# humanlongevity/tredparse

Measured on AMD Instinct MI355X. Metric: sample x TRED genotypes/sec at 30x 150bp, higher is better.
Workload: dtype int32 (SW) + f64 (likelihood)

## Files before the change

tredparse_amd/csrc/capi.hip:

```cpp
#include <algorithm>
#include <cstdarg>
#include <cstdio>
#include <cmath>
#include <cstdlib>
#include <cstring>
#include <ctime>
#include <string>
#include <vector>

#include <unistd.h>

#include "tredgpu_internal.h"
#include "inflater_internal.h"

using namespace tredgpu;

namespace {

struct Buf {
    void* p = nullptr;
    size_t cap = 0;
};

std::string g_create_error;

}

struct tredgpu_ctx {
    int device = 0;
    hipStream_t stream = nullptr;
    std::string err;
    std::vector<LadderDesc> h_ladders;
    Buf d_ladders, d_seq;
    int max_ladder_units = 0;
    Buf d_model;
    bool have_model = false;
    Buf ws_quads, ws_counter, ws_drop, ws_grid, ws_stats, ws_perm, ws_class, ws_gdesc, ws_gtile, ws_gctr, ws_ucnt, ws_bins, ws_kde, ws_best, ws_cnt;
    int* h_pin = nullptr;
    hipEvent_t sync_ev = nullptr;
    size_t grid_pool_bytes = GRID_POOL_BYTES;
    std::vector<Buf> st;
    struct PinBlock { uint8_t* p; size_t cap, used; };
    std::vector<PinBlock> pin;
    struct PinOut { void* host; const void* pinned; size_t bytes; };
    std::vector<PinOut> pin_out;
    struct Timer {
        std::vector<std::pair<hipEvent_t, hipEvent_t>> pool;
        size_t used = 0;
        int64_t launches = 0;
        double total_ms = 0;
    } timers[7];
};

namespace {

int fail(tredgpu_ctx* c, int code, const char* fmt, ...) {
    char buf[512];
    va_list ap;
    va_start(ap, fmt);
    vsnprintf(buf, sizeof buf, fmt, ap);
    va_end(ap);
    if (c) c->err = buf; else g_create_error = buf;
    return code;
}

int hip_rc(tredgpu_ctx* c, hipError_t e, const char* what) {
    return e == hipSuccess ? 0 : fail(c, -10, "%s: %s", what, hipGetErrorString(e));
}

#define HIPRC(c, expr) hip_rc((c), (expr), #expr)
#define HIPCHK(c, expr)                          \
    do {                                         \
        if (int rc_ = HIPRC(c, expr)) return rc_; \
    } while (0)

void timer_flush(tredgpu_ctx::Timer& t) {
    for (size_t i = 0; i < t.used; ++i) {
        float ms = 0;
        if (hipEventElapsedTime(&ms, t.pool[i].first, t.pool[i].second) == hipSuccess) {
            t.total_ms += ms;
            t.launches += 1;
        }
    }
    t.used = 0;
}

struct ScopedTimer {
    tredgpu_ctx* c;
    tredgpu_ctx::Timer& t;
    hipEvent_t stop = nullptr;
    ScopedTimer(tredgpu_ctx* c_, int which) : c(c_), t(c_->timers[which]) {
        if (t.used >= 256) {
            (void)hipStreamSynchronize(c->stream);
            timer_flush(t);
        }
        if (t.used == t.pool.size()) {
// ... 283 lines not shown
    if (!c || !out) return -2;
    HIPCHK(c, hipSetDevice(c->device));
    for (int i = 0; i < 8; ++i) out[i] = 0;
    if (c->ws_stats.p) {
        std::vector<uint64_t> slots((size_t)SW_STAT_SLOTS * 8);
        HIPCHK(c, hipMemcpyAsync(slots.data(), c->ws_stats.p, slots.size() * sizeof(uint64_t), hipMemcpyDeviceToHost, c->stream));
        HIPCHK(c, stream_sync(c));
        for (int k = 0; k < SW_STAT_SLOTS; ++k)
            for (int i = 0; i < 8; ++i) out[i] += slots[(size_t)k * 8 + i];
    }
    HIPCHK(c, stream_sync(c));
    return 0;
}

int tredgpu_get_timing(tredgpu_ctx* c, int which, int64_t* launches, double* total_ms) {
    if (!c) return -2;
    if (which < 0 || which > 6) return fail(c, -2, "which must be one of TREDGPU_KERNEL_*");
    HIPCHK(c, hipSetDevice(c->device));
    HIPCHK(c, stream_sync(c));
    timer_flush(c->timers[which]);
    if (launches) *launches = c->timers[which].launches;
    if (total_ms) *total_ms = c->timers[which].total_ms;
    return 0;
}

int tredgpu_set_ladders(tredgpu_ctx* c, int32_t n, const char* const* prefix, const char* const* repeat,
                        const char* const* suffix, const int32_t* max_units) {
    if (!c) return -2;
    if (n < 0 || (n > 0 && (!prefix || !repeat || !suffix || !max_units))) return fail(c, -2, "bad ladder arguments");
    HIPCHK(c, hipSetDevice(c->device));
    std::vector<uint32_t> seq;
    auto append = [&seq](const std::vector<int8_t>& v) {
        const int off = (int)seq.size();
        seq.resize(seq.size() + (v.size() + 7) / 8 + 1, 0x44444444u);
        for (size_t i = 0; i < v.size(); ++i) {
            uint32_t& w = seq[off + i / 8];
            w = (w & ~(0xFu << ((i % 8) * 4))) | ((uint32_t)v[i] << ((i % 8) * 4));
        }
        return off;
    };
    std::vector<LadderDesc> lad((size_t)n);
    int max_u = 0;
    for (int i = 0; i < n; ++i) {
        std::vector<int8_t> P, Rp, S;
        encode(prefix[i], P);
        encode(repeat[i], Rp);
        encode(suffix[i], S);
        const int mu = max_units[i];
        LadderDesc& d = lad[i];
        memset(&d, 0, sizeof d);
        if (mu < 0) return fail(c, -2, "ladder %d: negative max_units", i);
        if (mu == 0) {
            if (P.empty() || P.size() > TREDGPU_MAX_TEMPLATE_LEN)
                return fail(c, -2, "ladder %d: reference length %zu not in [1,%d]", i, P.size(), TREDGPU_MAX_TEMPLATE_LEN);
            d.alen[0] = (int)P.size();
            d.trunk_off[0] = append(P);
            d.branch_off[0] = append(std::vector<int8_t>());
            d.period = 1;
            d.max_units = 0;
            d.n_strands = 1;
            continue;
        }
        if (Rp.empty()) return fail(c, -2, "ladder %d: empty repeat", i);
        const size_t T = P.size() + S.size() + Rp.size() * (size_t)mu;
        if (T > TREDGPU_MAX_TEMPLATE_LEN)
            return fail(c, -2, "ladder %d: longest template %zu exceeds %d", i, T, TREDGPU_MAX_TEMPLATE_LEN);
        const std::vector<int8_t> Pr = revcomp(P), Rr = revcomp(Rp), Sr = revcomp(S);
        const std::vector<int8_t>* A[2] = {&P, &Sr};
        const std::vector<int8_t>* Rep[2] = {&Rp, &Rr};
        const std::vector<int8_t>* B[2] = {&S, &Pr};
        for (int s = 0; s < 2; ++s) {
            d.alen[s] = (int)A[s]->size();
            d.blen[s] = (int)B[s]->size();
            std::vector<int8_t> trunk(*A[s]);
            for (int k = 0; k < mu; ++k) trunk.insert(trunk.end(), Rep[s]->begin(), Rep[s]->end());
            d.trunk_off[s] = append(trunk);
            d.branch_off[s] = append(*B[s]);
        }
        d.period = (int)Rp.size();
        d.max_units = mu;
        d.n_strands = 2;
        d.kmer_ok = 1;
        for (int s = 0; s < 2; ++s) {
            std::vector<uint32_t> bits(128, 0u);
            for (int u = 1; u <= mu; ++u) {
                std::vector<int8_t> t(*A[s]);
                for (int k = 0; k < u; ++k) t.insert(t.end(), Rep[s]->begin(), Rep[s]->end());
                t.insert(t.end(), B[s]->begin(), B[s]->end());
                for (size_t i = 0; i + 6 <= t.size(); ++i) {
                    uint32_t code = 0;
                    int wild[6], nw = 0;
                    for (int k = 0; k < 6; ++k) {
                        if (t[i + k] > 3) wild[nw++] = k;
                        else code |= (uint32_t)(t[i + k] & 3) << (2 * k);
                    }
                    for (uint32_t f = 0; f < (1u << (2 * nw)); ++f) {
                        uint32_t cf = code;
                        for (int j = 0; j < nw; ++j) cf |= ((f >> (2 * j)) & 3u) << (2 * wild[j]);
                        bits[cf >> 5] |= 1u << (cf & 31);
                    }
                }
            }
            d.kmer_off[s] = (int)seq.size();
            seq.insert(seq.end(), bits.begin(), bits.end());
        }
        max_u = std::max(max_u, mu);
    }
    seq.resize(seq.size() + 4, 0x44444444u);
    int rc;
    if ((rc = ensure(c, c->d_ladders, lad.size() * sizeof(LadderDesc)))) return rc;
    if ((rc = ensure(c, c->d_seq, seq.size() * sizeof(uint32_t)))) return rc;
    HIPCHK(c, stream_sync(c));
    if (n) HIPCHK(c, hipMemcpy(c->d_ladders.p, lad.data(), lad.size() * sizeof(LadderDesc), hipMemcpyHostToDevice));
    HIPCHK(c, hipMemcpy(c->d_seq.p, seq.data(), seq.size() * sizeof(uint32_t), hipMemcpyHostToDevice));
    c->h_ladders.swap(lad);
    c->max_ladder_units = max_u;
    return 0;
}

int tredgpu_set_model(tredgpu_ctx* c, const double* step_pdf, const double* stutter_w, double gc, double score) {
    if (!c) return -2;
    if (!step_pdf || !stutter_w) return fail(c, -2, "model arrays are NULL");
    HIPCHK(c, hipSetDevice(c->device));
    std::vector<ModelConst> mbuf(1);
    ModelConst& m = mbuf[0];
    memcpy(m.step, step_pdf, sizeof m.step);
    memcpy(m.w, stutter_w, sizeof m.w);
    m.gc = gc;
    m.score = score;
    m.small = std::exp(-10.0);
    m.really_small = std::exp(-100.0);
    m.logsmall = std::log(m.small);
    for (int n = 0; n < GRID_LFACT; ++n) m.lfact[n] = std::lgamma((double)n + 1);
    int rc;
    if ((rc = ensure(c, c->d_model, sizeof m))) return rc;
    HIPCHK(c, stream_sync(c));
    HIPCHK(c, hipMemcpy(c->d_model.p, &m, sizeof m, hipMemcpyHostToDevice));
    c->have_model = true;
    return 0;
}

int64_t tredgpu_pack_reads(const char* seqs, const int64_t* seq_off, int64_t n_reads, uint32_t* packed_out,
                           int64_t* word_off_out, int32_t* len_out) {
    if (n_reads < 0 || (n_reads > 0 && (!seqs || !seq_off))) return -2;
    int64_t w = 0;
    for (int64_t r = 0; r < n_reads; ++r) {
        const int64_t L = seq_off[r + 1] - seq_off[r];
        if (L < 0 || L > 0x7fffffff) return -2;
        const int64_t nb = (L + 15) >> 4, nm = (L + 31) >> 5;
        if (word_off_out) word_off_out[r] = w;
        if (len_out) len_out[r] = (int32_t)L;
        if (packed_out) {
            uint32_t* rec = packed_out + w;
            for (int64_t k = 0; k < nb + nm; ++k) rec[k] = 0;
            const char* s = seqs + seq_off[r];
            for (int64_t i = 0; i < L; ++i) {
                const int code = base_code(s[i]);
                if (code == 4) rec[nb + (i >> 5)] |= 1u << (i & 31);
                else rec[i >> 4] |= (uint32_t)code << ((i & 15) * 2);
            }
        }
        w += nb + nm;
    }
    if (word_off_out) word_off_out[n_reads] = w;
    return w;
}


static int run_sw_device(tredgpu_ctx* c, const uint32_t* packed, const int64_t* read_off, const int32_t* read_len,
                         int64_t n_reads, const int32_t* unit_read_off, const int32_t* unit_ladder,
                         int32_t n_units, const tredgpu_sw_params* p, int max_len, uint8_t* out_tag,
                         int16_t* out_h, int16_t* out_score, int16_t* out_dump, int32_t dump_templates) {
    if (n_reads == 0 || n_units == 0) return 0;
    const int n_ladders = (int)c->h_ladders.size();
    const int64_t max_quads = sw_max_quads(n_reads, n_ladders);
    int rc;
    if ((rc = ensure(c, c->ws_quads, (size_t)max_quads * sizeof(Quad)))) return rc;
    if ((rc = ensure(c, c->ws_counter, 64))) return rc;
    SwArgs a;
    a.packed = packed;
    a.read_off = read_off;
    a.read_len = read_len;
    a.unit_read_off = unit_read_off;
    a.unit_ladder = unit_ladder;
    a.ladders = (const LadderDesc*)c->d_ladders.p;
    a.seqw = (const uint32_t*)c->d_seq.p;
    a.quads = (const Quad*)c->ws_quads.p;
    a.n_quads = (const int32_t*)c->ws_counter.p;
    a.out_tag = out_tag;
    a.out_h = out_h;
    a.out_score = out_score;
    a.out_dump = out_dump;
    a.dump_templates = dump_templates;
    a.n_units = n_units;
    a.n_ladders = n_ladders;
    a.max_rows = 16 * rows_for(max_len);
    a.p = *p;
    a.stats = nullptr;
    if ((rc = ensure(c, c->ws_perm, (size_t)n_reads * sizeof(int32_t)))) return rc;
    if ((rc = ensure(c, c->ws_class, (size_t)n_reads))) return rc;
    a.perm = (const int32_t*)c->ws_perm.p;
    if ((rc = ensure(c, c->ws_ucnt, sw_unit_cnt_bytes(n_units)))) return rc;
    if ((rc = ensure(c, c->ws_bins, sw_bin_bytes(n_ladders)))) return rc;
    if ((rc = ensure(c, c->ws_best, (size_t)n_reads * sizeof(int32_t)))) return rc;
    if ((rc = ensure(c, c->ws_cnt, (size_t)n_reads * sizeof(int32_t)))) return rc;
    a.best = (int32_t*)c->ws_best.p;
    if (c->ws_stats.p == nullptr) {
        if ((rc = ensure(c, c->ws_stats, SW_STAT_SLOTS * 8 * sizeof(unsigned long long)))) return rc;
        HIPCHK(c, hipMemsetAsync(c->ws_stats.p, 0, SW_STAT_SLOTS * 8 * sizeof(unsigned long long), c->stream));
    }
    a.stats = (unsigned long long*)c->ws_stats.p;
    const int rows = rows_for(max_len);
    auto build_quads = [&](int pass) {
        return launch_build_quads(a, pass, rows, (uint8_t*)c->ws_class.p, (int32_t*)c->ws_cnt.p, (int32_t*)c->ws_perm.p,
                                  (Quad*)c->ws_quads.p, (int32_t*)c->ws_counter.p, (int32_t*)c->ws_ucnt.p,
                                  (int32_t*)c->ws_bins.p, n_ladders, max_quads, c->stream);
    };
    HIPCHK(c, build_quads(0));
    {
        ScopedTimer tm(c, TREDGPU_KERNEL_SW);
        bool generic = false;
        bool two_strands = false;
        for (const LadderDesc& d : c->h_ladders) {
            for (int s2 = 0; s2 < d.n_strands; ++s2) generic = generic || (d.max_units > 0 && d.blen[s2] * p->match >= 30);
            two_strands = two_strands || d.n_strands >= 2;
        }
        HIPCHK(c, launch_sw_ladder(a, rows, generic, max_quads, c->stream));
        if (out_dump == nullptr && two_strands) {
            HIPCHK(c, build_quads(1));
            HIPCHK(c, launch_sw_ladder(a, rows, generic, max_quads, c->stream));
        }
    }
    return 0;
}

int tredgpu_sw_classify(tredgpu_ctx* c, int mem, const uint32_t* packed, const int64_t* read_off,
                        const int32_t* read_len, int64_t n_reads, const int32_t* unit_read_off,
                        const int32_t* unit_ladder, int32_t n_units, const tredgpu_sw_params* params,
                        uint8_t* out_tag, int16_t* out_h, int16_t* out_score, int16_t* out_dump,
                        int32_t dump_templates) {
    if (!c) return -2;
    int rc;
    if ((rc = check_sw_params(c, params))) return rc;
    if (n_reads < 0 || n_units < 0) return fail(c, -2, "negative sizes");
    if (n_reads > 0 && (!packed || !read_off || !read_len || !unit_read_off || !unit_ladder || !out_tag || !out_h || !out_score))
        return fail(c, -2, "NULL array argument");
    if (c->h_ladders.empty()) return fail(c, -4, "no ladders registered (tredgpu_set_ladders)");
    if (out_dump && dump_templates <= 0) return fail(c, -2, "dump_templates must be > 0 with out_dump");
    HIPCHK(c, hipSetDevice(c->device));
    int max_len = params->max_read_len;
    if (mem == TREDGPU_MEM_DEVICE) {
        if (max_len <= 0) max_len = TREDGPU_ASSUMED_READ_LEN;
        if (out_dump) HIPCHK(c, hipMemsetAsync(out_dump, 0xFF, (size_t)n_reads * dump_templates * 6 * sizeof(int16_t), c->stream));
        return run_sw_device(c, packed, read_off, read_len, n_reads, unit_read_off, unit_ladder, n_units, params,
                             max_len, out_tag, out_h, out_score, out_dump, dump_templates);
    }
    if (mem != TREDGPU_MEM_HOST) return fail(c, -2, "mem must be TREDGPU_MEM_HOST or TREDGPU_MEM_DEVICE");
    if (n_reads == 0) return 0;
    if (unit_read_off[0] != 0 || unit_read_off[n_units] != n_reads) return fail(c, -2, "unit_read_off must span [0,n_reads]");
    for (int g = 0; g < n_units; ++g) {
        if (unit_read_off[g + 1] < unit_read_off[g]) return fail(c, -2, "unit_read_off not monotone at %d", g);
        if (unit_ladder[g] < 0 || unit_ladder[g] >= (int)c->h_ladders.size()) return fail(c, -2, "unit %d: ladder %d not registered", g, unit_ladder[g]);
    }
    if ((rc = host_max_len(c, params, read_len, n_reads, &max_len))) return rc;
    const uint32_t* d_packed; const int64_t* d_off; const int32_t* d_len; const int32_t* d_uoff; const int32_t* d_ulad;
    uint8_t* d_tag; int16_t* d_h; int16_t* d_score; int16_t* d_dump = nullptr;
    const size_t n = (size_t)n_reads, g = (size_t)n_units, dump_n = out_dump ? n * dump_templates * 6 : 0;
    const std::vector<Staged> list = {
        arr_in(d_packed, packed, (size_t)read_off[n_reads]), arr_in(d_off, read_off, n + 1), arr_in(d_len, read_len, n),
        arr_in(d_uoff, unit_read_off, g + 1), arr_in(d_ulad, unit_ladder, g),
        arr_out(d_tag, out_tag, n), arr_out(d_h, out_h, n), arr_out(d_score, out_score, n),
        out_dump ? arr_out(d_dump, out_dump, dump_n) : absent,
    };
    rc = stage(c, list);
    if (!rc && out_dump) rc = HIPRC(c, hipMemsetAsync(d_dump, 0xFF, dump_n * sizeof(int16_t), c->stream));
    if (!rc) rc = run_sw_device(c, d_packed, d_off, d_len, n_reads, d_uoff, d_ulad, n_units, params, max_len, d_tag, d_h,
                                d_score, d_dump, dump_templates);
    return finish(c, list, rc);
}

int tredgpu_tally(tredgpu_ctx* c, int mem, const uint8_t* tag, const int16_t* h, int64_t n_reads,
                  const int32_t* unit_read_off, int32_t n_units, const int32_t* read_pair_id, int32_t hist_stride,
                  int32_t* full_cnt, int32_t* pref_cnt, int32_t* rept_cnt) {
    if (!c) return -2;
    if (n_reads < 0 || n_units < 0 || hist_stride <= 0) return fail(c, -2, "bad sizes");
    if (n_units > 0 && (!unit_read_off || !full_cnt || !pref_cnt || !rept_cnt)) return fail(c, -2, "NULL array argument");
    if (n_reads > 0 && (!tag || !h)) return fail(c, -2, "NULL array argument");
    HIPCHK(c, hipSetDevice(c->device));
    int rc;
// ... 402 lines not shown
```

tredparse_amd/csrc/sw_ladder.hip:

```cpp
#include "tredgpu_internal.h"

namespace tredgpu {
namespace {

constexpr int KSH = 18;
constexpr int KONE = 1 << KSH;
constexpr int PAYMASK = KONE - 1;
constexpr int NEG = -(1 << 30);
constexpr int PADNEG = -64 * KONE;

template <int CTRL>
__device__ __forceinline__ int dpp_row_shr(int old, int x) {
    return __builtin_amdgcn_update_dpp(old, x, CTRL, 0xF, 0xF, false);
}

__device__ __forceinline__ int add3_vsv(int v0, int s1, int v2) {
    int d;
    asm("v_add3_u32 %0, %1, %2, %3" : "=v"(d) : "v"(v0), "s"(s1), "v"(v2));
    return d;
}
__device__ __forceinline__ int add_sv(int s0, int v1) {
    int d;
    asm("v_add_u32 %0, %1, %2" : "=v"(d) : "s"(s0), "v"(v1));
    return d;
}
__device__ __forceinline__ int max3(int a, int b, int c) { return max(max(a, b), c); }

__device__ __forceinline__ int row_scan_max(int x) {
    x = max(x, dpp_row_shr<0x111>(x, x));
    x = max(x, dpp_row_shr<0x112>(x, x));
    x = max(x, dpp_row_shr<0x114>(x, x));
    x = max(x, dpp_row_shr<0x118>(x, x));
    return x;
}

template <int CTRL>
__device__ __forceinline__ void pair_step(int& k, int& s) {
    const int tk = dpp_row_shr<CTRL>(k, k);
    const int ts = dpp_row_shr<CTRL>(s, s);
    const bool c = tk > k;
    k = c ? tk : k;
    s = c ? ts : s;
}

template <int R>
struct Rows {
    int S[4][R];
    int rowc0;
};

struct Track {
    int bestkey;
    int beststart;
    int ceil;
};

__device__ __forceinline__ int row_excl_scan_max(int x) {
    constexpr int IMIN = -2147483647 - 1;
    x = max(x, dpp_row_shr<0x111>(IMIN, x));
    x = max(x, dpp_row_shr<0x112>(IMIN, x));
    x = max(x, dpp_row_shr<0x114>(IMIN, x));
    x = max(x, dpp_row_shr<0x118>(IMIN, x));
    return dpp_row_shr<0x111>(NEG, x);
}

__device__ __forceinline__ int row_max_all(int x) {
    constexpr int IMIN = -2147483647 - 1;
    x = max(x, __builtin_amdgcn_update_dpp(IMIN, x, 0x121, 0xF, 0xF, false));
    x = max(x, __builtin_amdgcn_update_dpp(IMIN, x, 0x122, 0xF, 0xF, false));
    x = max(x, __builtin_amdgcn_update_dpp(IMIN, x, 0x124, 0xF, 0xF, false));
    x = max(x, __builtin_amdgcn_update_dpp(IMIN, x, 0x128, 0xF, 0xF, false));
    return x;
}

__device__ __forceinline__ int row_scan_max_fused(int x) {
    constexpr int IMIN = -2147483647 - 1;
    x = max(x, dpp_row_shr<0x111>(IMIN, x));
    x = max(x, dpp_row_shr<0x112>(IMIN, x));
    x = max(x, dpp_row_shr<0x114>(IMIN, x));
    x = max(x, dpp_row_shr<0x118>(IMIN, x));
    return x;
}

__device__ __forceinline__ int row_excl_scan_max_e10(int x, int* E, const int* q, int before) {
    int fin;
    asm("v_max_i32 %2, %2, %12\n\t"
        "v_max_i32 %3, %3, %13\n\t"
        "v_max_i32_dpp %0, %0, %0 row_shr:1 row_mask:0xf bank_mask:0xf\n\t"
        "v_max_i32 %4, %4, %14\n\t"
        "v_max_i32 %5, %5, %15\n\t"
        "v_max_i32_dpp %0, %0, %0 row_shr:2 row_mask:0xf bank_mask:0xf\n\t"
        "v_max_i32 %6, %6, %16\n\t"
// ... 244 lines not shown

__device__ __forceinline__ int lane_now() {
    int l;
    asm volatile("v_mbcnt_lo_u32_b32 %0, -1, 0\n\tv_mbcnt_hi_u32_b32 %0, -1, %0" : "=v"(l));
    return l;
}

#ifndef SW_WAVES_R4
#define SW_WAVES_R4 6
#endif
#ifndef SW_WAVES_R7
#define SW_WAVES_R7 6
#endif
#ifndef SW_WAVES_R10
#define SW_WAVES_R10 4
#endif
#ifndef SW_WAVES_R16
#define SW_WAVES_R16 3
#endif
#ifndef SW_WAVES_R20
#define SW_WAVES_R20 2
#endif
#ifndef SW_WAVES_R32
#define SW_WAVES_R32 1
#endif
template <int R, int W, bool GENERIC>
__global__ __launch_bounds__(64, W) void sw_cont_kernel(SwArgs a) {
    constexpr int PS = 64;
    __shared__ __attribute__((aligned(8))) int wbuf[(3 * R + 2) * PS + 2 * PS];
    const int lane = threadIdx.x;
    const int64_t q = (int64_t)blockIdx.x;
    const int nq = *a.n_quads;
    if (q >= nq) return;
    const int q_ladder = __builtin_amdgcn_readfirstlane(a.quads[q].ladder);
    const int q_first = __builtin_amdgcn_readfirstlane(a.quads[q].first);
    const int q_strands = __builtin_amdgcn_readfirstlane(a.quads[q].strands);
    const int q_count = __builtin_amdgcn_readfirstlane(a.quads[q].count);
    const LadderDesc* ld = a.ladders + q_ladder;
    const int period = __builtin_amdgcn_readfirstlane(ld->period);
    const int max_units = __builtin_amdgcn_readfirstlane(ld->max_units);
    const int n_strands = __builtin_amdgcn_readfirstlane(ld->n_strands);

    const int job = lane >> 4, jl = lane & 15;
    const bool valid = job < q_count;
    int L, row0;
    bool too_long;
    int best;
    {
        const int64_t rd = valid ? (int64_t)a.perm[q_first + job] : 0;
        L = valid ? a.read_len[rd] : 0;
        best = valid ? a.best[rd] : -1;
        too_long = L > 16 * R;
        if (too_long) L = 0;
        row0 = jl * R;
    }
    auto read_base = [&]() -> int64_t {
        const int jb = lane_now() >> 4;
        return jb < q_count ? a.read_off[a.perm[q_first + jb]] : 0;
    };
    const int mK = a.p.match * KONE;
    const int xK = -a.p.mismatch * KONE;
    const int geK = a.p.gap_extend * KONE;
    const int c0 = (a.p.gap_open - a.p.gap_extend) * KONE;
    const int flank = a.p.flank;
    const bool full_dump = GENERIC && a.out_dump != nullptr;
    int* const wb = wbuf + lane;
    int* const rowbuf = wb + (2 * R + 2) * PS;

    const int mu_rept = a.p.clip ? (L + period - 1) / period : max_units;

    uint32_t cnt_cols = 0, cnt_ends = 0;

    const int kmer_thr = min(a.p.mismatch, a.p.gap_open) >= 5 * a.p.match ? (30 + a.p.match - 1) / a.p.match - 5 : 0;
    const int floor_key = (full_dump ? 0 : 29) << KSH | PAYMASK;

    for (int s = 0; s < n_strands; ++s) {
        if (!((q_strands >> s) & 1)) continue;
        const int trunk_w = __builtin_amdgcn_readfirstlane(ld->trunk_off[s]);
        const int alen = __builtin_amdgcn_readfirstlane(ld->alen[s]);
        const int blen = __builtin_amdgcn_readfirstlane(ld->blen[s]);
        const int ncols = alen + period * max_units;
        int kcap = 1 << 20;
        if constexpr (R >= 5 && 2 * R + 10 <= 32) if (!full_dump && kmer_thr > 0 && __builtin_amdgcn_readfirstlane(ld->kmer_ok) != 0) {
            const uint32_t* bm = a.seqw + __builtin_amdgcn_readfirstlane(ld->kmer_off[s]);
            uint32_t pk_s, nk_s;
            {
                int L_s = L, row0_s = row0;
                asm volatile("" : "+v"(L_s), "+v"(row0_s));
                uint64_t code2;
                uint32_t nmask;
                load_rows<R>(a, read_base(), L_s, row0_s, code2, nmask);
                const int n_real = min(max(L_s - row0_s, 0), R);
                pk_s = (uint32_t)code2 & ((1u << (2 * R)) - 1u);
                nk_s = (nmask | ~((1u << n_real) - 1u)) & ((1u << R) - 1u);
            }
            const uint32_t pk_n = (uint32_t)__builtin_amdgcn_update_dpp(0, (int)pk_s, 0x101, 0xF, 0xF, false);
            const uint32_t nk_n = (uint32_t)__builtin_amdgcn_update_dpp(0x3FF, (int)nk_s, 0x101, 0xF, 0xF, false);
            const uint32_t comb = pk_s | ((pk_n & 0x3FFu) << (2 * R));
            const uint32_t ncomb = nk_s | ((nk_n & 0x1Fu) << R);
            int cnt = 0;
#pragma unroll
            for (int r = 0; r < R; ++r) {
                const uint32_t win = (comb >> (2 * r)) & 0xFFFu;
                const bool has_n = ((ncomb >> r) & 0x3Fu) != 0;
                const bool in_read = row0 + r + 5 < L;
                const uint32_t word = bm[win >> 5];
                cnt += in_read && (has_n || ((word >> (win & 31)) & 1u));
            }
            cnt += dpp_row_shr<0x111>(0, cnt);
            cnt += dpp_row_shr<0x112>(0, cnt);
            cnt += dpp_row_shr<0x114>(0, cnt);
            cnt += dpp_row_shr<0x118>(0, cnt);
            kcap = (cnt + 5) * a.p.match;
            if (__builtin_amdgcn_ballot_w64(valid && jl == 15 && cnt >= kmer_thr) == 0) continue;
        }
        const int cap = min(kcap, L * a.p.match);
        auto still_open = [&](int un) {
            const int min_score = max(min(L, alen + period * un + blen) >> 1, 30);
            return max(min_score, (best >> 12) + 1) <= cap;
        };
        if (!full_dump && __builtin_amdgcn_ballot_w64(valid && jl == 15 && still_open(max_units > 0 ? 1 : 0)) == 0) continue;

        Rows<R> J;
        int H[R], E[R];
        const bool has_suffix = max_units > 0 && blen > 0;
        if (has_suffix) {
            build_profile<R>(J, a, read_base(), L, row0, true, mK, xK, geK);
            const int branch_w = __builtin_amdgcn_readfirstlane(ld->branch_off[s]);
            const int ln = lane_now();
            const int bw = ln < ((blen + 7) >> 3) ? (int)a.seqw[branch_w + ln] : 0;
            int D[R];
#pragma unroll
            for (int r = 0; r < R; ++r) { H[r] = NEG; E[r] = NEG; }
            for (int y = 0; y + 1 < blen; ++y) {
                const int s_fresh = (y << 9) + y * geK - 2 * geK;
                switch (letter_from(bw, blen - 1 - y)) {
                    case 0: sweep_column_free<R, 0>(J, H, E, s_fresh, geK, c0); break;
                    case 1: sweep_column_free<R, 1>(J, H, E, s_fresh, geK, c0); break;
                    case 2: sweep_column_free<R, 2>(J, H, E, s_fresh, geK, c0); break;
                    case 3: sweep_column_free<R, 3>(J, H, E, s_fresh, geK, c0); break;
                    default: sweep_column_free<R, 4>(J, H, E, s_fresh, geK, c0); break;
                }
            }
            {
                const int y = blen - 1;
                const int s_fresh = (y << 9) + y * geK - 2 * geK;
                switch (letter_from(bw, 0)) {
                    case 0: match_column<R, 0>(J, H, D, s_fresh, geK); break;
                    case 1: match_column<R, 1>(J, H, D, s_fresh, geK); break;
                    case 2: match_column<R, 2>(J, H, D, s_fresh, geK); break;
                    case 3: match_column<R, 3>(J, H, D, s_fresh, geK); break;
                    default: match_column<R, 4>(J, H, D, s_fresh, geK); break;
                }
            }
            mirror_up<R>(D, 0, wb, PS);
            mirror_up<R>(E, c0, wb + R * PS, PS);
#pragma unroll
            for (int r = 0; r < R; ++r) wb[r * PS] = max(wb[r * PS], wb[(R + r) * PS] - c0);
            cnt_cols += (uint32_t)blen << 16;
        }
        build_profile<R>(J, a, read_base(), L, row0, false, mK, xK, geK);
        const int row0g = row0 * geK;
        Track T;
        const bool with_sfx = GENERIC && has_suffix && (full_dump || blen * a.p.match >= 30);
        if (with_sfx) {
            const int branch_w = __builtin_amdgcn_readfirstlane(ld->branch_off[s]);
            const int ln = lane_now();
            const int bw = ln < ((blen + 7) >> 3) ? (int)a.seqw[branch_w + ln] : 0;
            column_start<R>(J, H, E, geK);
            T.bestkey = floor_key; T.beststart = 0; T.ceil = floor_key;
            for (int j = 0; j < blen; ++j) sweep_letter<R>(letter_from(bw, j), J, H, E, T, j, row0, geK, c0, row0g, rowbuf);
            resolve_best<R>(T, row0, row0g, geK, rowbuf);
            int sk = T.bestkey, ss = T.beststart;
            pair_step<0x111>(sk, ss);
            pair_step<0x112>(sk, ss);
            pair_step<0x114>(sk, ss);
            pair_step<0x118>(sk, ss);
            wb[(2 * R) * PS] = sk;
            wb[(2 * R + 1) * PS] = ss;
        }
        const int ln_t = lane_now();
        const int tw = ln_t < ((ncols + 7) >> 3) ? (int)a.seqw[trunk_w + ln_t] : 0;
        column_start<R>(J, H, E, geK);
        T.bestkey = floor_key; T.beststart = 0; T.ceil = floor_key;
        int next_end = max_units > 0 ? alen + period - 1 : alen - 1;
        int u = max_units > 0 ? 1 : 0;
        auto template_end = [&](int col) -> bool {
            const bool comb = blen > 0;
            const int Tlen = alen + period * u + blen;
            next_end += period;
            int bk, bs;
            if (comb) {
                long long* const slot = reinterpret_cast<long long*>(wbuf + (3 * R + 2) * PS) + lane_now();
#pragma unroll
                for (int r0 = 0; r0 < R; r0 += END_CHUNK<R>) {
                    int wh[END_CHUNK<R>], we[END_CHUNK<R>];
// ... 76 lines not shown
                const int k = max_units > 0 ? 2 * (u - 1) + s : 0;
                if (k < a.dump_templates) {
                    int16_t* d = a.out_dump + ((int64_t)a.perm[q_first + job] * a.dump_templates + k) * 6;
                    const bool hit = score > 0 && bk != floor_key;
                    d[0] = (int16_t)(hit ? score : 0);
                    d[1] = (int16_t)(hit ? ref_begin : -1);
                    d[2] = (int16_t)(hit ? ref_end : -1);
                    d[3] = (int16_t)(hit ? read_begin : 0);
                    d[4] = (int16_t)(hit ? read_end : 0);
                    d[5] = (int16_t)tag;
                }
            }
            ++u;
            if (!full_dump && __builtin_amdgcn_ballot_w64(valid && jl == 15 && still_open(u)) == 0) return true;
            return false;
        };
        int ok_run = 0;
        auto steady_exit = [&](const uint32_t ends_before) -> bool {
            if (full_dump || ((cnt_ends ^ ends_before) & 0xFF00u) == 0) { ok_run = 0; return false; }
            const uint32_t thr = (uint32_t)(alen + (ok_run ? period : 0)) << 9;
            uint32_t lo = 0x3FFFFu;
#pragma unroll
            for (int r = 0; r < R; ++r) lo = min(lo, min((uint32_t)H[r] & 0x3FE00u, (uint32_t)E[r] & 0x3FE00u));
            if (__builtin_amdgcn_ballot_w64(lo < thr) != 0) { ok_run = 0; return false; }
            if (ok_run) return true;
            ok_run = 1;
            return false;
        };
        if (period == 3 && max_units > 0) {
            int col = 0;
            for (; col < alen; ++col) {
                sweep_letter<R>(letter_from(tw, col), J, H, E, T, col, row0, geK, c0, row0g, rowbuf);
                ++cnt_cols;
            }
            int P0[R], P1[R], P2[R];
            pick_profile<R>(J, letter_from(tw, alen), geK, P0);
            pick_profile<R>(J, letter_from(tw, alen + 1), geK, P1);
            pick_profile<R>(J, letter_from(tw, alen + 2), geK, P2);
            for (;;) {
                sweep_at<R>(J, P0, H, E, T, col, row0, geK, c0, row0g, rowbuf);
                sweep_at<R>(J, P1, H, E, T, col + 1, row0, geK, c0, row0g, rowbuf);
                sweep_at<R>(J, P2, H, E, T, col + 2, row0, geK, c0, row0g, rowbuf);
                col += 3;
                cnt_cols += 3;
                const uint32_t ends_before = cnt_ends;
                if (template_end(col - 1) || col >= ncols || steady_exit(ends_before)) break;
            }
        } else {
            for (int col = 0; col < ncols; ++col) {
                sweep_letter<R>(letter_from(tw, col), J, H, E, T, col, row0, geK, c0, row0g, rowbuf);
                ++cnt_cols;
                if (col != next_end) continue;
                const uint32_t ends_before = cnt_ends;
                if (template_end(col) || (max_units > 0 && steady_exit(ends_before))) break;
            }
        }
    }
    const int lane_e = lane_now();
    if (a.stats != nullptr && lane_e < 7) {
        const int n_trunk_cols = (int)(cnt_cols & 0xFFFFu), n_cont_cols = (int)(cnt_cols >> 16);
        const int vals[7] = {n_trunk_cols, n_cont_cols, (int)(cnt_ends & 0xFFu), (int)((cnt_ends >> 8) & 0xFFu),
                             (int)(cnt_ends >> 16), 1, (n_trunk_cols + n_cont_cols) * q_count};
        int v = 0;
#pragma unroll
        for (int k = 0; k < 7; ++k) v = lane_e == k ? vals[k] : v;
        atomicAdd(a.stats + (size_t)(blockIdx.x & (SW_STAT_SLOTS - 1)) * 8 + lane_e, (unsigned long long)v);
    }
    if ((lane_e >> 4) < q_count && (lane_e & 15) == 15) {
        const int64_t rd = (int64_t)a.perm[q_first + (lane_e >> 4)];
        int bestTag = best < 0 ? TREDGPU_TAG_NONE : best & 7;
        int bestU = 511 - ((best >> 3) & 511), bestS = best >> 12;
        if (too_long) bestTag = TREDGPU_TAG_INVALID, bestU = 0, bestS = 0;
        a.out_tag[rd] = (uint8_t)bestTag;
        a.out_h[rd] = (int16_t)(bestTag == TREDGPU_TAG_NONE ? 0 : bestU);
        a.out_score[rd] = (int16_t)(bestTag == TREDGPU_TAG_NONE ? 0 : bestS);
        a.best[rd] = best;
    }
}

constexpr int BIN_STRIDE = 16;
constexpr int SW_LEVELS = 32;
constexpr int UNIT_BINS = SW_LEVELS;
constexpr int KEY_NONE = 0xFF;
constexpr int CNT_UNFILTERED = 0x7FFF;
__device__ __forceinline__ int level_key(int cnt) { return SW_LEVELS - 1 - min(SW_LEVELS - 1, cnt / 6); }
__device__ __forceinline__ int kmer_threshold(const tredgpu_sw_params& p) {
    return min(p.mismatch, p.gap_open) >= 5 * p.match ? (30 + p.match - 1) / p.match - 5 : 0;
}

__device__ __forceinline__ void claim_bin_runs(const int* hist, int lad, int g, int32_t* unit_cnt, int32_t* bin_total) {
    for (int k = threadIdx.x; k < UNIT_BINS; k += (int)blockDim.x) {
        const int n = hist[k];
        int at = 0;
        if (n) at = atomicAdd(bin_total + ((size_t)lad * UNIT_BINS + k) * BIN_STRIDE, n);
        unit_cnt[(size_t)g * UNIT_BINS + k] = at;
    }
}

__device__ __forceinline__ void kmer_counts(const uint32_t* rec, int L, const uint32_t* bm, int& cnt0, int& cnt1) {
    const int nb = (L + 15) >> 4;
    uint32_t prev = 0, mprev = 0;
    cnt0 = cnt1 = 0;
    for (int wi = 0; wi < nb; ++wi) {
        const uint32_t w = rec[wi];
        const uint32_t m = (rec[nb + (wi >> 1)] >> ((wi & 1) * 16)) & 0xffffu;
        uint32_t b0 = 0, b1 = 0;
#pragma unroll
        for (int j = 0; j < 16; ++j) {
            const uint32_t t = j > 5 ? w >> (2 * (j - 5)) : (j == 5 ? w : __builtin_amdgcn_alignbit(w, prev, 32 - 2 * (5 - j)));
            const uint32_t at = __builtin_amdgcn_ubfe(t, 5, 7);
            b0 = (__builtin_amdgcn_ubfe(bm[at], t, 1) << j) | b0;
            b1 = (__builtin_amdgcn_ubfe(bm[128 + at], t, 1) << j) | b1;
        }
        const uint32_t mm = m << 5 | mprev >> 11;
        const uint32_t hn = mm | mm >> 1 | mm >> 2 | mm >> 3 | mm >> 4 | mm >> 5;
        const int left = L - wi * 16;
        uint32_t cm = left >= 16 ? 0xffffu : (1u << left) - 1u;
        if (wi == 0) cm &= ~0x1fu;
        cnt0 += __builtin_popcount((b0 | hn) & cm);
        cnt1 += __builtin_popcount((b1 | hn) & cm);
        prev = w;
        mprev = m;
    }
}

__global__ __launch_bounds__(64) void read_class_kernel(SwArgs a, uint8_t* read_key, int32_t* read_cnt, int32_t* unit_cnt,
                                                          int32_t* bin_total) {
    const int g = blockIdx.x;
    if (g >= a.n_units) return;
    const int lad = min(max(a.unit_ladder[g], 0), a.n_ladders - 1);
    const LadderDesc* ld = a.ladders + lad;
    const bool full_dump = a.out_dump != nullptr;
    const int thr = kmer_threshold(a.p);
    const bool filt = !full_dump && thr > 0 && ld->kmer_ok != 0 && ld->max_units > 0;
    const int r0 = a.unit_read_off[g], r1 = a.unit_read_off[g + 1];
    __shared__ uint32_t bm[2][128];
    __shared__ int hist[UNIT_BINS];
    if (filt) {
        for (int k = threadIdx.x; k < 256; k += (int)blockDim.x) bm[k >> 7][k & 127] = a.seqw[ld->kmer_off[k >> 7] + (k & 127)];
    }
    for (int k = threadIdx.x; k < UNIT_BINS; k += (int)blockDim.x) hist[k] = 0;
    __syncthreads();
    for (int rd = r0 + (int)threadIdx.x; rd < r1; rd += (int)blockDim.x) {
        int cnt0 = CNT_UNFILTERED, cnt1 = CNT_UNFILTERED;
        const int L = a.read_len[rd];
        if (filt && L <= a.max_rows) kmer_counts(a.packed + a.read_off[rd], L, &bm[0][0], cnt0, cnt1);
        read_cnt[rd] = cnt0 | cnt1 << 16;
        a.best[rd] = -1;
        if (cnt0 >= thr) {
            const int key = level_key(cnt0);
            read_key[rd] = (uint8_t)key;
            atomicAdd(&hist[key], 1);
        } else {
            read_key[rd] = (uint8_t)KEY_NONE;
            a.out_tag[rd] = TREDGPU_TAG_NONE;
            a.out_h[rd] = 0;
            a.out_score[rd] = 0;
        }
    }
    __syncthreads();
    claim_bin_runs(hist, lad, g, unit_cnt, bin_total);
}

__global__ __launch_bounds__(64) void repack_kernel(SwArgs a, uint8_t* read_key, const int32_t* read_cnt, int32_t* unit_cnt,
                                                      int32_t* bin_total, int kcap_in_kernel) {
    const int g = blockIdx.x;
    if (g >= a.n_units) return;
    const int lad = min(max(a.unit_ladder[g], 0), a.n_ladders - 1);
    const LadderDesc* ld = a.ladders + lad;
    const int thr = kmer_threshold(a.p);
    const bool with_kcap = kcap_in_kernel && thr > 0 && ld->kmer_ok != 0;
    const bool two_strands = ld->n_strands >= 2;
    const int first_T = ld->alen[1] + ld->period * (ld->max_units > 0 ? 1 : 0) + ld->blen[1];
    const int r0 = a.unit_read_off[g], r1 = a.unit_read_off[g + 1];
    __shared__ int hist[UNIT_BINS];
    __shared__ int n_pass;
    for (int k = threadIdx.x; k < UNIT_BINS; k += (int)blockDim.x) hist[k] = 0;
    if (threadIdx.x == 0) n_pass = 0;
    __syncthreads();
    for (int rd = r0 + (int)threadIdx.x; rd < r1; rd += (int)blockDim.x) {
        const int L = a.read_len[rd];
        const int cnt1 = (int)((uint32_t)read_cnt[rd] >> 16);
        const bool counted = cnt1 != CNT_UNFILTERED;
        const int kcap = with_kcap && counted ? (cnt1 + 5) * a.p.match : 1 << 20;
        const int cap = min(kcap, L * a.p.match);
        const int min_score = max(min(L, first_T) >> 1, 30);
        const bool open = max(min_score, (a.best[rd] >> 12) + 1) <= cap;
        const bool go = two_strands && L <= a.max_rows && cnt1 >= thr && open;
        int key = KEY_NONE;
        if (go) {
            key = level_key(cnt1);
            atomicAdd(&hist[key], 1);
            atomicAdd(&n_pass, 1);
        }
        read_key[rd] = (uint8_t)key;
    }
    __syncthreads();
    claim_bin_runs(hist, lad, g, unit_cnt, bin_total);
    if (threadIdx.x == 0 && a.stats != nullptr && n_pass)
        atomicAdd(a.stats + (size_t)(g & (SW_STAT_SLOTS - 1)) * 8 + 7, (unsigned long long)n_pass);
}

__global__ __launch_bounds__(1024) void bin_scan_kernel(int32_t* bins, int n_bins, int32_t* n_quads) {
    __shared__ int cs[1024], cq[1024];
    const int t = threadIdx.x;
    const int chunk = (n_bins + 1023) / 1024;
    const int b0 = min(t * chunk, n_bins), b1 = min(b0 + chunk, n_bins);
    int slots = 0, quads = 0;
    for (int b = b0; b < b1; ++b) {
        const int n = bins[(size_t)b * BIN_STRIDE];
        slots += n;
        quads += (n + 3) >> 2;
    }
    cs[t] = slots; cq[t] = quads;
    __syncthreads();
    if (t == 0) {
        int s = 0, q = 0;
        for (int k = 0; k < 1024; ++k) { const int a_ = cs[k], b_ = cq[k]; cs[k] = s; cq[k] = q; s += a_; q += b_; }
        bins[(size_t)n_bins * BIN_STRIDE + 2] = q;
        *n_quads = q;
    }
    __syncthreads();
    int slot = cs[t], quad = cq[t];
    for (int b = b0; b < b1; ++b) {
        int32_t* e = bins + (size_t)b * BIN_STRIDE;
        e[1] = slot;
        e[2] = quad;
        slot += e[0];
        quad += (e[0] + 3) >> 2;
    }
}

__global__ __launch_bounds__(64) void scatter_kernel(SwArgs a, const uint8_t* read_key, const int32_t* unit_cnt, int32_t* bins,
                                                       int32_t* perm) {
    const int g = blockIdx.x;
    if (g >= a.n_units) return;
    const int lad = min(max(a.unit_ladder[g], 0), a.n_ladders - 1);
    __shared__ int pos[UNIT_BINS];
    for (int k = threadIdx.x; k < UNIT_BINS; k += (int)blockDim.x)
        pos[k] = bins[((size_t)lad * UNIT_BINS + k) * BIN_STRIDE + 1] + unit_cnt[(size_t)g * UNIT_BINS + k];
    __syncthreads();
    const int r0 = a.unit_read_off[g], r1 = a.unit_read_off[g + 1];
    for (int r = r0 + (int)threadIdx.x; r < r1; r += (int)blockDim.x) {
        const int key = read_key[r];
        if (key != KEY_NONE) perm[atomicAdd(&pos[key], 1)] = r;
    }
}

__global__ void fill_quads_kernel(const int32_t* bins, int n_bins, const int32_t* n_quads, Quad* quads,
                                  const LadderDesc* ladders, int strand_mask) {
    const int q = blockIdx.x * blockDim.x + threadIdx.x;
    if (q >= *n_quads) return;
    int lo = 0, hi = n_bins;
    while (hi - lo > 1) {
        const int mid = (lo + hi) >> 1;
        if (bins[(size_t)mid * BIN_STRIDE + 2] <= q) lo = mid; else hi = mid;
    }
    const int32_t* e = bins + (size_t)lo * BIN_STRIDE;
    const int j = q - e[2];
    Quad qd;
    qd.ladder = lo / UNIT_BINS;
    qd.first = e[1] + 4 * j;
    qd.count = min(4, e[0] - 4 * j);
    qd.strands = strand_mask & (ladders[qd.ladder].n_strands >= 2 ? 3 : 1);
    quads[q] = qd;
}

// ... 132 lines not shown
```

tredparse_amd/csrc/tredgpu_internal.h:

```cpp
#pragma once
#include <hip/hip_runtime.h>
#include <stdint.h>
#include "../../include/tredgpu.h"

namespace tredgpu {

struct LadderDesc {
    int32_t alen[2];
    int32_t blen[2];
    int32_t trunk_off[2];
    int32_t branch_off[2];
    int32_t period;
    int32_t max_units;
    int32_t n_strands;
    int32_t kmer_ok;
    int32_t kmer_off[2];
};

struct Quad {
    int32_t ladder;
    int32_t first;
    int32_t count;
    int32_t strands;
};

struct SwArgs {
    const uint32_t* packed;
    const int64_t* read_off;
    const int32_t* read_len;
    const int32_t* unit_read_off;
    const int32_t* unit_ladder;
    const LadderDesc* ladders;
    const uint32_t* seqw;
    const Quad* quads;
    const int32_t* perm;
    const int32_t* n_quads;
    uint8_t* out_tag;
    int16_t* out_h;
    int16_t* out_score;
    int16_t* out_dump;
    int32_t dump_templates;
    int32_t n_units;
    int32_t n_ladders;
    int32_t max_rows;
    tredgpu_sw_params p;
    unsigned long long* stats;
    int32_t* best;
};

constexpr int SW_STAT_SLOTS = 1024;

hipError_t launch_build_quads(const SwArgs& a, int pass, int rows_per_lane, uint8_t* read_key, int32_t* read_cnt, int32_t* perm,
                              Quad* quads, int32_t* n_quads, int32_t* unit_cnt, int32_t* bins, int n_ladders, int64_t max_quads,
                              hipStream_t s);
size_t sw_bin_bytes(int n_ladders);
size_t sw_unit_cnt_bytes(int n_units);
int64_t sw_max_quads(int64_t n_reads, int n_ladders);
hipError_t launch_sw_ladder(const SwArgs& a, int rows_per_lane, bool generic, int64_t max_quads, hipStream_t s);
hipError_t launch_tally(const uint8_t* tag, const int16_t* h, int64_t n_reads,
                        const int32_t* unit_read_off, int32_t n_units, const int32_t* read_pair_id,
                        int32_t hist_stride, int32_t* full_cnt, int32_t* pref_cnt,
                        int32_t* rept_cnt, uint8_t* scratch_drop, hipStream_t s);

struct ModelConst {
    double step[6][37];
    double w[5];
    double gc, score;
    double small;
    double really_small;
    double logsmall;
    double lfact[4096];
};
constexpr int GRID_LFACT = 4096;

struct GridArgs {
    const tredgpu_unit_params* units;
    int32_t n_units;
    int32_t hist_stride;
    const int32_t* full_cnt;
    const int32_t* pref_cnt;
    const int32_t* rept_cnt;
    const int32_t* global_lens;
    const int32_t* target_lens;
    tredgpu_call* calls;
    const int64_t* grid_off;
    double* grid_dump;
    double* marg;
    int32_t marg_stride;
    const ModelConst* model;
    const int64_t* joint_off;
    double* joint;
    int32_t* joint_n;
    double* joint_total;
    double* kde_pdf;
    int32_t* kde_status;
    double* unit_pdf;
    int32_t* unit_kde_rc;
    int32_t max_target;
};
constexpr int GRID_MAX_ROWS = 1024;
constexpr int GRID_MAX_COLS = 1024;
constexpr size_t GRID_POOL_BYTES = (size_t)12 << 30;
constexpr int GRID_UNIT_DEFERRED = 100;

hipError_t launch_pe_kde(const GridArgs& a, hipStream_t s);
hipError_t launch_unit_max(const tredgpu_unit_params* units, int n_units, int* out, hipStream_t s);
size_t grid_desc_bytes();
size_t grid_counter_bytes();
int grid_deferred_offset();
size_t grid_slot_doubles_max(int rows_cap, int cols_cap, int nt_max);
size_t grid_items_cap(int rows_cap, int cols_cap);
size_t grid_item_bytes();
size_t grid_item_slots(int n_units, int rows_cap, int cols_cap);
int grid_subpools(size_t pool_doubles, int rows_cap, int cols_cap, int nt_max);
size_t grid_units_per_subpool(int n_units, int n_sub);
hipError_t launch_grid_pass(const GridArgs& a, int pass, void* descs, double* pool, size_t pool_doubles, int rows_cap,
                            int cols_cap, void* items, size_t item_cap, void* counters, hipStream_t s, int phases = 15);

}
```

Before: 1.504 million.

## Reuse precomputed k-mer counts in SW kernel and tighten N-wildcard bounds

The SW ladder kernel no longer recomputes per-read 6-mer hit counts with DPP reductions. It reads the counts the quad-builder already wrote to the read_cnt workspace, indexed through the permutation. For templates containing N bases, a new per-kmer table of the fewest wildcards needed is built on the host and used to subtract a weight from the count, which tightens the score cap and prunes more reads. The host table build also deduplicates repeated kmer keys. The risk is an extra gather from global memory per quad and more shared memory in the count kernel.

```diff
diff --git a/tredparse_amd/csrc/capi.hip b/tredparse_amd/csrc/capi.hip
--- a/tredparse_amd/csrc/capi.hip
+++ b/tredparse_amd/csrc/capi.hip
@@ -12,6 +12,7 @@
 
 #include "tredgpu_internal.h"
 #include "inflater_internal.h"
+#include "kmer_host.h"
 
 using namespace tredgpu;
 
@@ -461,27 +462,15 @@
         d.n_strands = 2;
         d.kmer_ok = 1;
         for (int s = 0; s < 2; ++s) {
-            std::vector<uint32_t> bits(128, 0u);
-            for (int u = 1; u <= mu; ++u) {
-                std::vector<int8_t> t(*A[s]);
-                for (int k = 0; k < u; ++k) t.insert(t.end(), Rep[s]->begin(), Rep[s]->end());
-                t.insert(t.end(), B[s]->begin(), B[s]->end());
-                for (size_t i = 0; i + 6 <= t.size(); ++i) {
-                    uint32_t code = 0;
-                    int wild[6], nw = 0;
-                    for (int k = 0; k < 6; ++k) {
-                        if (t[i + k] > 3) wild[nw++] = k;
-                        else code |= (uint32_t)(t[i + k] & 3) << (2 * k);
-                    }
-                    for (uint32_t f = 0; f < (1u << (2 * nw)); ++f) {
-                        uint32_t cf = code;
-                        for (int j = 0; j < nw; ++j) cf |= ((f >> (2 * j)) & 3u) << (2 * wild[j]);
-                        bits[cf >> 5] |= 1u << (cf & 31);
-                    }
-                }
-            }
+            std::vector<uint32_t> bits, cls;
+            const bool with_n = kmer_host::build_tables(*A[s], *Rep[s], *B[s], mu, bits, cls);
             d.kmer_off[s] = (int)seq.size();
             seq.insert(seq.end(), bits.begin(), bits.end());
+            d.kmer_n = with_n ? 1 : 0;
+            if (with_n) {
+                d.kcls_off[s] = (int)seq.size();
+                seq.insert(seq.end(), cls.begin(), cls.end());
+            }
         }
         max_u = std::max(max_u, mu);
     }
@@ -584,6 +573,7 @@
     if ((rc = ensure(c, c->ws_best, (size_t)n_reads * sizeof(int32_t)))) return rc;
     if ((rc = ensure(c, c->ws_cnt, (size_t)n_reads * sizeof(int32_t)))) return rc;
     a.best = (int32_t*)c->ws_best.p;
+    a.read_cnt = (const int32_t*)c->ws_cnt.p;
     if (c->ws_stats.p == nullptr) {
         if ((rc = ensure(c, c->ws_stats, SW_STAT_SLOTS * 8 * sizeof(unsigned long long)))) return rc;
         HIPCHK(c, hipMemsetAsync(c->ws_stats.p, 0, SW_STAT_SLOTS * 8 * sizeof(unsigned long long), c->stream));
diff --git a/tredparse_amd/csrc/kmer_host.h b/tredparse_amd/csrc/kmer_host.h
--- /dev/null
+++ b/tredparse_amd/csrc/kmer_host.h
@@ -0,0 +1,56 @@
+#pragma once
+#include <cstdint>
+#include <vector>
+
+namespace kmer_host {
+
+constexpr int BITS_WORDS = 128;
+constexpr int CLS_WORDS = 512;
+
+template <class Vec>
+inline bool holds_n(const Vec& v) {
+    for (size_t i = 0; i < v.size(); ++i)
+        if (v[i] > 3) return true;
+    return false;
+}
+
+template <class Vec>
+inline bool build_tables(const Vec& head, const Vec& repeat, const Vec& branch, int max_units, std::vector<uint32_t>& bits,
+                         std::vector<uint32_t>& cls) {
+    bits.assign(BITS_WORDS, 0u);
+    cls.clear();
+    const bool with_n = max_units > 0 && (holds_n(head) || holds_n(repeat) || holds_n(branch));
+    std::vector<uint8_t> fewest(4096, 15);
+    std::vector<bool> seen((size_t)1 << 18, false);
+    Vec t;
+    for (int u = 1; u <= max_units; ++u) {
+        t.assign(head.begin(), head.end());
+        for (int k = 0; k < u; ++k) t.insert(t.end(), repeat.begin(), repeat.end());
+        t.insert(t.end(), branch.begin(), branch.end());
+        for (size_t i = 0; i + 6 <= t.size(); ++i) {
+            uint32_t code = 0, mask = 0;
+            int wild[6], nw = 0;
+            for (int k = 0; k < 6; ++k) {
+                if (t[i + k] > 3) { wild[nw++] = k; mask |= 1u << k; }
+                else code |= (uint32_t)(t[i + k] & 3) << (2 * k);
+            }
+            const uint32_t key = code | mask << 12;
+            if (seen[key]) continue;
+            seen[key] = true;
+            for (uint32_t f = 0; f < (1u << (2 * nw)); ++f) {
+                uint32_t cf = code;
+                for (int j = 0; j < nw; ++j) cf |= ((f >> (2 * j)) & 3u) << (2 * wild[j]);
+                bits[cf >> 5] |= 1u << (cf & 31);
+                if (nw < fewest[cf]) fewest[cf] = (uint8_t)nw;
+            }
+        }
+    }
+    if (with_n) {
+        cls.assign(CLS_WORDS, 0u);
+        for (uint32_t w = 0; w < 4096; ++w)
+            if (fewest[w] != 15) cls[w >> 3] |= (uint32_t)fewest[w] << (4 * (w & 7));
+    }
+    return with_n;
+}
+
+}
diff --git a/tredparse_amd/csrc/sw_ladder.hip b/tredparse_amd/csrc/sw_ladder.hip
--- a/tredparse_amd/csrc/sw_ladder.hip
+++ b/tredparse_amd/csrc/sw_ladder.hip
@@ -8,6 +8,10 @@
 constexpr int PAYMASK = KONE - 1;
 constexpr int NEG = -(1 << 30);
 constexpr int PADNEG = -64 * KONE;
+constexpr int CNT_UNFILTERED = 0x7FFF;
+
+__device__ __forceinline__ int kmer_weight(int cnt, int jsum) { return cnt - (jsum + 5) / 6; }
+__device__ __forceinline__ int kmer_cap(int w, int match) { return (w + 5) * match; }
 
 template <int CTRL>
 __device__ __forceinline__ int dpp_row_shr(int old, int x) {
@@ -418,36 +422,9 @@
         const int ncols = alen + period * max_units;
         int kcap = 1 << 20;
         if constexpr (R >= 5 && 2 * R + 10 <= 32) if (!full_dump && kmer_thr > 0 && __builtin_amdgcn_readfirstlane(ld->kmer_ok) != 0) {
-            const uint32_t* bm = a.seqw + __builtin_amdgcn_readfirstlane(ld->kmer_off[s]);
-            uint32_t pk_s, nk_s;
-            {
-                int L_s = L, row0_s = row0;
-                asm volatile("" : "+v"(L_s), "+v"(row0_s));
-                uint64_t code2;
-                uint32_t nmask;
-                load_rows<R>(a, read_base(), L_s, row0_s, code2, nmask);
-                const int n_real = min(max(L_s - row0_s, 0), R);
-                pk_s = (uint32_t)code2 & ((1u << (2 * R)) - 1u);
-                nk_s = (nmask | ~((1u << n_real) - 1u)) & ((1u << R) - 1u);
-            }
-            const uint32_t pk_n = (uint32_t)__builtin_amdgcn_update_dpp(0, (int)pk_s, 0x101, 0xF, 0xF, false);
-            const uint32_t nk_n = (uint32_t)__builtin_amdgcn_update_dpp(0x3FF, (int)nk_s, 0x101, 0xF, 0xF, false);
-            const uint32_t comb = pk_s | ((pk_n & 0x3FFu) << (2 * R));
-            const uint32_t ncomb = nk_s | ((nk_n & 0x1Fu) << R);
-            int cnt = 0;
-#pragma unroll
-            for (int r = 0; r < R; ++r) {
-                const uint32_t win = (comb >> (2 * r)) & 0xFFFu;
-                const bool has_n = ((ncomb >> r) & 0x3Fu) != 0;
-                const bool in_read = row0 + r + 5 < L;
-                const uint32_t word = bm[win >> 5];
-                cnt += in_read && (has_n || ((word >> (win & 31)) & 1u));
-            }
-            cnt += dpp_row_shr<0x111>(0, cnt);
-            cnt += dpp_row_shr<0x112>(0, cnt);
-            cnt += dpp_row_shr<0x114>(0, cnt);
-            cnt += dpp_row_shr<0x118>(0, cnt);
-            kcap = (cnt + 5) * a.p.match;
+            const int jb = lane_now() >> 4;
+            const int cnt = jb < q_count ? (int)reinterpret_cast<const uint16_t*>(a.read_cnt)[2 * (int64_t)a.perm[q_first + jb] + s] : 0;
+            if (cnt != CNT_UNFILTERED) kcap = kmer_cap(cnt, a.p.match);
             if (__builtin_amdgcn_ballot_w64(valid && jl == 15 && cnt >= kmer_thr) == 0) continue;
         }
         const int cap = min(kcap, L * a.p.match);
@@ -690,7 +667,6 @@
 constexpr int SW_LEVELS = 32;
 constexpr int UNIT_BINS = SW_LEVELS;
 constexpr int KEY_NONE = 0xFF;
-constexpr int CNT_UNFILTERED = 0x7FFF;
 __device__ __forceinline__ int level_key(int cnt) { return SW_LEVELS - 1 - min(SW_LEVELS - 1, cnt / 6); }
 __device__ __forceinline__ int kmer_threshold(const tredgpu_sw_params& p) {
     return min(p.mismatch, p.gap_open) >= 5 * p.match ? (30 + p.match - 1) / p.match - 5 : 0;
@@ -705,30 +681,43 @@
     }
 }
 
-__device__ __forceinline__ void kmer_counts(const uint32_t* rec, int L, const uint32_t* bm, int& cnt0, int& cnt1) {
+template <bool NCLS>
+__device__ __forceinline__ void kmer_counts(const uint32_t* rec, int L, const uint32_t* bm, const uint32_t* kc, int& cnt0, int& cnt1) {
     const int nb = (L + 15) >> 4;
     uint32_t prev = 0, mprev = 0;
     cnt0 = cnt1 = 0;
+    int j0 = 0, j1 = 0;
     for (int wi = 0; wi < nb; ++wi) {
         const uint32_t w = rec[wi];
         const uint32_t m = (rec[nb + (wi >> 1)] >> ((wi & 1) * 16)) & 0xffffu;
         uint32_t b0 = 0, b1 = 0;
+        const uint32_t mm = m << 5 | mprev >> 11;
+        const uint32_t hn = mm | mm >> 1 | mm >> 2 | mm >> 3 | mm >> 4 | mm >> 5;
+        const int left = L - wi * 16;
+        uint32_t cm = left >= 16 ? 0xffffu : (1u << left) - 1u;
+        if (wi == 0) cm &= ~0x1fu;
+        const uint32_t plain = cm & ~hn;
 #pragma unroll
         for (int j = 0; j < 16; ++j) {
             const uint32_t t = j > 5 ? w >> (2 * (j - 5)) : (j == 5 ? w : __builtin_amdgcn_alignbit(w, prev, 32 - 2 * (5 - j)));
             const uint32_t at = __builtin_amdgcn_ubfe(t, 5, 7);
             b0 = (__builtin_amdgcn_ubfe(bm[at], t, 1) << j) | b0;
             b1 = (__builtin_amdgcn_ubfe(bm[128 + at], t, 1) << j) | b1;
-        }
-        const uint32_t mm = m << 5 | mprev >> 11;
-        const uint32_t hn = mm | mm >> 1 | mm >> 2 | mm >> 3 | mm >> 4 | mm >> 5;
-        const int left = L - wi * 16;
-        uint32_t cm = left >= 16 ? 0xffffu : (1u << left) - 1u;
-        if (wi == 0) cm &= ~0x1fu;
+            if (NCLS) {
+                const uint32_t at4 = __builtin_amdgcn_ubfe(t, 3, 9), sh = (t & 7u) << 2;
+                const bool use = (plain >> j) & 1u;
+                j0 += use ? (int)__builtin_amdgcn_ubfe(kc[at4], sh, 4) : 0;
+                j1 += use ? (int)__builtin_amdgcn_ubfe(kc[512 + at4], sh, 4) : 0;
+            }
+        }
         cnt0 += __builtin_popcount((b0 | hn) & cm);
         cnt1 += __builtin_popcount((b1 | hn) & cm);
         prev = w;
         mprev = m;
+    }
+    if (NCLS) {
+        cnt0 = kmer_weight(cnt0, j0);
+        cnt1 = kmer_weight(cnt1, j1);
     }
 }
 
@@ -743,16 +732,24 @@
     const bool filt = !full_dump && thr > 0 && ld->kmer_ok != 0 && ld->max_units > 0;
     const int r0 = a.unit_read_off[g], r1 = a.unit_read_off[g + 1];
     __shared__ uint32_t bm[2][128];
+    __shared__ uint32_t kc[2][512];
     __shared__ int hist[UNIT_BINS];
+    const bool ncls = filt && ld->kmer_n != 0;
     if (filt) {
         for (int k = threadIdx.x; k < 256; k += (int)blockDim.x) bm[k >> 7][k & 127] = a.seqw[ld->kmer_off[k >> 7] + (k & 127)];
+    }
+    if (ncls) {
+        for (int k = threadIdx.x; k < 1024; k += (int)blockDim.x) kc[k >> 9][k & 511] = a.seqw[ld->kcls_off[k >> 9] + (k & 511)];
     }
     for (int k = threadIdx.x; k < UNIT_BINS; k += (int)blockDim.x) hist[k] = 0;
     __syncthreads();
     for (int rd = r0 + (int)threadIdx.x; rd < r1; rd += (int)blockDim.x) {
         int cnt0 = CNT_UNFILTERED, cnt1 = CNT_UNFILTERED;
         const int L = a.read_len[rd];
-        if (filt && L <= a.max_rows) kmer_counts(a.packed + a.read_off[rd], L, &bm[0][0], cnt0, cnt1);
+        if (filt && L <= a.max_rows) {
+            if (ncls) kmer_counts<true>(a.packed + a.read_off[rd], L, &bm[0][0], &kc[0][0], cnt0, cnt1);
+            else kmer_counts<false>(a.packed + a.read_off[rd], L, &bm[0][0], nullptr, cnt0, cnt1);
+        }
         read_cnt[rd] = cnt0 | cnt1 << 16;
         a.best[rd] = -1;
         if (cnt0 >= thr) {
@@ -790,7 +787,7 @@
         const int L = a.read_len[rd];
         const int cnt1 = (int)((uint32_t)read_cnt[rd] >> 16);
         const bool counted = cnt1 != CNT_UNFILTERED;
-        const int kcap = with_kcap && counted ? (cnt1 + 5) * a.p.match : 1 << 20;
+        const int kcap = with_kcap && counted ? kmer_cap(cnt1, a.p.match) : 1 << 20;
         const int cap = min(kcap, L * a.p.match);
         const int min_score = max(min(L, first_T) >> 1, 30);
         const bool open = max(min_score, (a.best[rd] >> 12) + 1) <= cap;
diff --git a/tredparse_amd/csrc/tredgpu_internal.h b/tredparse_amd/csrc/tredgpu_internal.h
--- a/tredparse_amd/csrc/tredgpu_internal.h
+++ b/tredparse_amd/csrc/tredgpu_internal.h
@@ -15,6 +15,8 @@
     int32_t n_strands;
     int32_t kmer_ok;
     int32_t kmer_off[2];
+    int32_t kmer_n;
+    int32_t kcls_off[2];
 };
 
 struct Quad {
@@ -46,6 +48,7 @@
     tredgpu_sw_params p;
     unsigned long long* stats;
     int32_t* best;
+    const int32_t* read_cnt;
 };
 
 constexpr int SW_STAT_SLOTS = 1024;
```

Result: faster. 1.655 million, median of 6 (+10.0%).
